# LUP-LuftbildUmweltPlanung/UNet

Measured on AMD Instinct MI355X. Metric: 512x512 tiles/sec fwd+bwd (4-ch->5-class U-Net), higher is better.
Workload: dtype f32

## Files before the change

### include/unet_hip.h

```cpp
#ifndef UNET_HIP_H
#define UNET_HIP_H

#include <stddef.h>
#include <stdint.h>

#ifdef __cplusplus
extern "C" {
#endif

#define UNET_OK 0
#define UNET_E_BADARG (-1)
#define UNET_E_UNSUPPORTED (-2)
#define UNET_E_HIP (-3)

#define UNET_ABI_VERSION 8

int unet_abi_version(void);
const char* unet_last_error(void);

#define UNET_F32 0
#define UNET_BF16 1
typedef uint16_t unet_bf16;

typedef struct {
// ... 48 lines not shown
    int ps_tail_c, ps_tail_at;
} unet_conv_desc;

int unet_conv2d_colsum_rows(const unet_conv_desc* d);
int unet_conv2d(const unet_conv_desc* d, void* stream);
size_t unet_conv2d_splitk_workspace(const unet_conv_desc* d);
int unet_conv2d_variant(const unet_conv_desc* d);
size_t unet_pack_weights_size(int Cout, int Cin, int ks, int mode);
int unet_pack_weights(const float* w, float* wp, int Cout, int Cin, int ks, int mode, void* stream);
int unet_pack_weights_strided(const float* w, long long so, long long sr, float* wp, int O, int R, void* stream);
size_t unet_pack_weights_size_bf16(int Cout, int Cin, int ks, int mode);
int unet_pack_weights_bf16(const float* w, unet_bf16* wp, int Cout, int Cin, int ks, int mode, void* stream);
typedef struct {
    const float* w;
    void* wp;
    int Cout, Cin, ks, mode;
    const float* out_scale;
} unet_pack_job;
size_t unet_pack_batch_table_bytes(int njobs);
int unet_pack_batch_build(const unet_pack_job* jobs, int njobs, int dtype, void* table_host, unsigned* total_blocks);
int unet_pack_batch_run(const void* table_dev, int njobs, unsigned total_blocks, int dtype, void* stream);
typedef struct {
    const float* x; int x_cs, x_co;
    const float* dy; int dy_cs, dy_co;
    float* dw;
    float* dbias;
    int N, IH, IW, Cin, OH, OW, Cout, ks, stride;
    float* workspace; size_t workspace_floats;
    int accumulate;
    int dtype;
    const unet_tuning* tuning;
} unet_wgrad_desc;
size_t unet_conv2d_wgrad_workspace(const unet_wgrad_desc* d);
int unet_conv2d_wgrad(const unet_wgrad_desc* d, void* stream);

int unet_bn_stats_rows(long long P);
int unet_bn_stats(const float* x, int x_cs, int x_co, long long P, int C, float* partial, void* stream);
int unet_bn_finalize(const float* psum, const float* psumsq, int rows, long long count, int C,
                     const float* gamma, const float* beta, float* running_mean, float* running_var,
                     float momentum, float eps,
                     float* scale, float* shift, float* save_mean, float* save_invstd, long long* batches_tracked, void* stream);
int unet_bn_eval_coeffs(const float* gamma, const float* beta, const float* running_mean, const float* running_var,
                        float eps, int C, float* scale, float* shift, void* stream);
int unet_affine_act(const float* x, int x_cs, int x_co, const float* scale, const float* shift,
                    const float* x2, int x2_cs, int x2_co, const float* scale2, const float* shift2,
                    float* y, int y_cs, int y_co, long long P, int C, int relu, void* stream);
int unet_bn_bwd_reduce(const float* dout, int d_cs, int d_co, const float* out, int o_cs, int o_co,
                       const float* x, int x_cs, int x_co, const float* mean, const float* invstd,
                       long long P, int C, float* partial, void* stream);
int unet_bn_bwd_finalize(const float* partial, int rows, long long count, int C,
                         float* dgamma, float* dbeta, float* c1, float* c2, void* stream);
int unet_bn_bwd_apply(const float* dout, int d_cs, int d_co, const float* out, int o_cs, int o_co,
                      const float* x, int x_cs, int x_co, const float* mean, const float* invstd,
                      const float* gamma, const float* c1, const float* c2,
                      float* dx, int dx_cs, int dx_co, float* gout, int g_cs, int g_co, int g_accumulate,
                      long long P, int C, void* stream);

int unet_maxpool3x3s2(const float* x, int x_cs, int x_co, float* y, int y_cs, int y_co, uint8_t* idx,
                      int N, int IH, int IW, int C, int OH, int OW, void* stream);
int unet_maxpool3x3s2_bwd(const float* dy, int dy_cs, int dy_co, const uint8_t* idx, float* dx, int dx_cs, int dx_co,
                          int N, int IH, int IW, int C, int OH, int OW, int accumulate, void* stream);
int unet_avgpool2_ceil(const float* x, int x_cs, int x_co, float* y, int y_cs, int y_co,
                       int N, int IH, int IW, int C, int OH, int OW, void* stream);
int unet_avgpool2_ceil_bwd(const float* dy, int dy_cs, int dy_co, float* dx, int dx_cs, int dx_co,
                           int N, int IH, int IW, int C, int OH, int OW, int accumulate, void* stream);

// ... 304 lines not shown
```

### unet_amd/_lib.py

```python
from __future__ import annotations

import ctypes as C
import os
import re
from pathlib import Path

import torch

_HERE = Path(__file__).resolve().parent
LIB_PATH = _HERE / "lib" / "libunet_hip.so"
HEADER = _HERE.parent / "include" / "unet_hip.h"

UNET_OK = 0
CONV_RELU = 1
CONV_MASK = 4
CONV_FWD = 0
CONV_DGRAD = 1
F32 = 0
BF16 = 1

c_float_p = C.POINTER(C.c_float)
vp = C.c_void_p


# ... 100 lines not shown

def _load() -> C.CDLL:
    if not LIB_PATH.exists():
        raise ImportError(
            f"{LIB_PATH} not found: build it with `python -m unet_amd.build` (hipcc --offload-arch=gfx950). "
            "The MI355X path has no CPU fallback.")
    lib = C.CDLL(str(LIB_PATH))
    missing = [s for s in declared_symbols() if not hasattr(lib, s)]
    if missing:
        raise ImportError(f"libunet_hip.so does not export: {missing}")
    return lib


lib = _load()

i, ll, f, sz = C.c_int, C.c_longlong, C.c_float, C.c_size_t
_sig = {
    "unet_abi_version": (i, []),
    "unet_last_error": (C.c_char_p, []),
    "unet_conv2d_colsum_rows": (i, [C.POINTER(ConvDesc)]),
    "unet_conv2d": (i, [C.POINTER(ConvDesc), vp]),
    "unet_conv2d_variant": (i, [C.POINTER(ConvDesc)]),
    "unet_conv2d_splitk_workspace": (sz, [C.POINTER(ConvDesc)]),
    "unet_tuning_default": (None, [C.POINTER(Tuning)]),
    "unet_pack_batch_table_bytes": (sz, [i]),
    "unet_pack_batch_build": (i, [C.POINTER(PackJob), i, i, vp, C.POINTER(C.c_uint)]),
    "unet_pack_batch_run": (i, [vp, i, C.c_uint, i, vp]),
    "unet_pack_weights_size": (sz, [i, i, i, i]),
    "unet_pack_weights": (i, [vp, vp, i, i, i, i, vp]),
    "unet_pack_weights_strided": (i, [vp, ll, ll, vp, i, i, vp]),
    "unet_row_softmax": (i, [vp, i, i, vp, i, i, ll, i, vp]),
    "unet_row_softmax_bwd": (i, [vp, i, i, vp, i, i, vp, i, i, ll, i, vp]),
    "unet_conv2d_wgrad_workspace": (sz, [C.POINTER(WgradDesc)]),
    "unet_conv2d_wgrad": (i, [C.POINTER(WgradDesc), vp]),
    "unet_bn_stats_rows": (i, [ll]),
    "unet_bn_stats": (i, [vp, i, i, ll, i, vp, vp]),
    "unet_bn_finalize": (i, [vp, vp, i, ll, i, vp, vp, vp, vp, f, f, vp, vp, vp, vp, vp, vp]),
    "unet_bn_eval_coeffs": (i, [vp, vp, vp, vp, f, i, vp, vp, vp]),
    "unet_affine_act": (i, [vp, i, i, vp, vp, vp, i, i, vp, vp, vp, i, i, ll, i, i, vp]),
    "unet_bn_bwd_reduce": (i, [vp, i, i, vp, i, i, vp, i, i, vp, vp, ll, i, vp, vp]),
    "unet_bn_bwd_finalize": (i, [vp, i, ll, i, vp, vp, vp, vp, vp]),
    "unet_bn_bwd_apply": (i, [vp, i, i, vp, i, i, vp, i, i, vp, vp, vp, vp, vp, vp, i, i, vp, i, i, i, ll, i, vp]),
    "unet_maxpool3x3s2": (i, [vp, i, i, vp, i, i, vp, i, i, i, i, i, i, vp]),
    "unet_maxpool3x3s2_bwd": (i, [vp, i, i, vp, vp, i, i, i, i, i, i, i, i, i, vp]),
    "unet_avgpool2_ceil": (i, [vp, i, i, vp, i, i, i, i, i, i, i, i, vp]),
    "unet_avgpool2_ceil_bwd": (i, [vp, i, i, vp, i, i, i, i, i, i, i, i, i, vp]),
    "unet_shuffle_blur": (i, [vp, i, i, vp, i, i, i, i, i, i, i, vp]),
    "unet_shuffle_blur_bwd": (i, [vp, i, i, vp, i, i, vp, i, i, i, i, i, i, i, vp]),
    "unet_shuffle_bwd_xmask": (i, [vp, i, i, vp, i, i, vp, i, i, i, i, i, i, vp]),
    "unet_resize_nearest": (i, [vp, i, i, vp, i, i, i, i, i, i, i, i, vp]),
    "unet_resize_nearest_bwd": (i, [vp, i, i, vp, i, i, i, i, i, i, i, i, vp]),
    "unet_nchw_to_nhwc": (i, [vp, vp, i, i, i, i, i, i, vp]),
    "unet_nhwc_to_nchw": (i, [vp, i, i, vp, i, i, i, i, vp]),
    "unet_copy_slice": (i, [vp, i, i, vp, i, i, ll, i, i, vp]),
    "unet_relu_mask": (i, [vp, i, i, vp, i, i, vp, i, i, ll, i, vp]),
    "unet_colsum": (i, [vp, i, i, ll, i, vp, vp, vp]),
    "unet_colsum_workspace": (sz, [ll, i]),
    "unet_dot": (i, [vp, i, i, vp, i, i, ll, i, vp, vp, vp]),
    "unet_ce_workspace": (sz, [ll]),
    "unet_ce_fwd": (i, [vp, i, i, vp, vp, ll, i, vp, vp, vp, vp]),
    "unet_ce_fwd_parts": (i, [vp, i, i, vp, vp, ll, i, vp, vp, vp]),
    "unet_ce_bwd": (i, [vp, i, i, vp, vp, ll, i, vp, f, vp, i, i, vp]),
    "unet_ce_fwd_pw": (i, [vp, i, i, vp, vp, ll, i, vp, vp, vp, vp]),
    "unet_ce_fwd_parts_pw": (i, [vp, i, i, vp, vp, ll, i, vp, vp, vp]),
    "unet_ce_bwd_pw": (i, [vp, i, i, vp, vp, ll, i, vp, f, vp, i, i, vp]),
    "unet_focal_fwd": (i, [vp, i, i, vp, vp, ll, i, f, vp, vp, vp]),
# ... 133 lines not shown
```

### unet_amd/csrc/conv_wgrad.hip

```cpp

#include <type_traits>
#include <utility>

#include "common.h"

namespace {

template <typename F, int... Is>
__device__ __forceinline__ void static_for_impl(F&& f, std::integer_sequence<int, Is...>) { (f(std::integral_constant<int, Is>{}), ...); }
template <int N, typename F>
__device__ __forceinline__ void static_for(F&& f) { static_for_impl(f, std::make_integer_sequence<int, N>{}); }


typedef float f32x16 __attribute__((ext_vector_type(16)));

constexpr int BK = 64;
constexpr int BC = 64;

struct WArgs {
    const float* x; const float* dy; float* part;
    float* bpart;
    int x_cs, x_co, dy_cs, dy_co;
    int N, IH, IW, Cin, Cin4, OH, OW, Cout, Cout4;
    int tiles_y, tiles_x, total_tiles, tiles_per_block;
    int kt, ct;
    int cw, nnb;
    int xcd_map;
    int csub, ksub;
};

template <int PTW, int S, int KS>
__global__ __launch_bounds__(256, 2) void wgrad_kernel(const WArgs a) {
    constexpr int PT = (S == 1) ? 64 : 32;
    constexpr int PTH = PT / PTW;
    constexpr int PAD = (KS - 1) / 2;
    constexpr int T = KS * KS;
    constexpr int HH = (PTH - 1) * S + KS, HW = (PTW - 1) * S + KS, HPIX = HH * HW;
// ... 259 lines not shown
            for (int p = 0; p < PT; ++p) bsum += dyT[p * LD + tid];
        }
#ifdef UNET_WGRAD16_NOSKIP
        compute(T1{}, T1{});
#else
        if (mv0 && nv0) {
            if (mv1 && nv1) compute(T1{}, T1{});
            else if (mv1) compute(T1{}, T0{});
            else if (nv1) compute(T0{}, T1{});
            else compute(T0{}, T0{});
        }
#endif
        __syncthreads();
    }

    if (do_bias && k0 + tid < a.Cout) a.bpart[(size_t)split * a.Cout + k0 + tid] = bsum;
    const size_t KC_ = (size_t)a.Cout * a.Cin;
    float* pb = a.part + (size_t)split * T * KC_;
#pragma unroll
    for (int i = 0; i < 2; ++i)
#pragma unroll
        for (int j = 0; j < 2; ++j) {
            const int c = c0 + wc * 32 + 16 * j + l15;
#pragma unroll
            for (int t = 0; t < T; ++t)
#pragma unroll
                for (int r = 0; r < 4; ++r) {
                    const int k = k0 + wk * 32 + 16 * i + 4 * kq + r;
                    if (k < a.Cout && c < a.Cin) pb[(size_t)t * KC_ + (size_t)k * a.Cin + c] = acc[i][j][t][r];
                }
        }
}

template <int KT, int NTW, bool SLV = false>
__global__ __launch_bounds__(256, 2) void wgrad_flat_kernel(const WArgs a) {
    constexpr int PT = 32, HW = 34, HPIX = 3 * HW, LD = 112, Q = LD / 4;
    constexpr int DIT = (PT * Q + 255) / 256, XIT = (HPIX * Q + 255) / 256;
    typedef float f32x4 __attribute__((ext_vector_type(4)));
    extern __shared__ __attribute__((aligned(16))) float smem[];
    float* dyT = smem;
    float* xh = smem + PT * LD;

    const int tid = threadIdx.x, lane = tid & 63, wave = __builtin_amdgcn_readfirstlane(tid >> 6);
    const int l15 = lane & 15, kk = lane >> 4;
    const int cols = gridDim.x;
    const int lin = blockIdx.x + cols * blockIdx.y;
    const int xcd = lin & 7, qq = lin >> 3;
    const int bx = qq % cols, split = xcd + 8 * (qq / cols);
    const int chunk = bx / a.nnb, nb = bx % a.nnb;
    const int c0 = chunk * a.cw;
    const int CW = (a.Cin - c0) < a.cw ? (a.Cin - c0) : a.cw;
    const int NTOT = 9 * CW;
    const int tile_begin = split * a.tiles_per_block;
    int tile_end = tile_begin + a.tiles_per_block;
    if (tile_end > a.total_tiles) tile_end = a.total_tiles;
    if (tile_begin >= a.total_tiles) return;

    int bfix[NTW], brow[NTW];
#pragma unroll
    for (int q = 0; q < NTW; ++q) {
        const int n = ((nb * 4 + wave) * NTW + q) * 16 + l15;
        const int nn = n < NTOT ? n : 0;
        const int t = nn / CW, c = nn - t * CW;
        const int r = t / 3, s_ = t - 3 * r;
        bfix[q] = (s_ + kk) * LD + c;
        brow[q] = r;
    }
    const int abase = kk * LD + l15;
    const int sbase = kk * LD + 16 * KT + (l15 & 3);

    f32x4 acc[KT][NTW];
    f32x4 sacc[SLV ? NTW : 1];
#pragma unroll
    for (int m = 0; m < KT; ++m)
#pragma unroll
        for (int q = 0; q < NTW; ++q) acc[m][q] = (f32x4){0.f, 0.f, 0.f, 0.f};
#pragma unroll
    for (int q = 0; q < (SLV ? NTW : 1); ++q) sacc[q] = (f32x4){0.f, 0.f, 0.f, 0.f};

    constexpr bool PF = (KT * NTW + (SLV ? NTW : 0) <= 36);
    constexpr int RIT = (HW * Q + 255) / 256;
    const int cw4 = (CW + 3) & ~3;
    struct TilePos { int oy, ox0; const float* dyb; const float* xb; };
    auto tile_pos = [&](int tile) {
        int b = tile;
        TilePos t;
        t.oy = b % a.OH; b /= a.OH;
        const int tx = b % a.tiles_x;
        const int img = b / a.tiles_x;
        t.ox0 = tx * PT;
        t.dyb = a.dy + ((size_t)img * a.OH + t.oy) * a.OW * a.dy_cs + a.dy_co;
        t.xb = a.x + (size_t)img * a.IH * a.IW * a.x_cs + a.x_co + c0;
        return t;
    };
    auto load_dy = [&](const TilePos& t, float4 (&r)[DIT]) {
#pragma unroll
        for (int it = 0; it < DIT; ++it) {
            const int e = tid + it * 256;
            const int p = e / Q, q = e - p * Q;
            const bool ok = (e < PT * Q) && (t.ox0 + p) < a.OW && 4 * q < a.Cout4;
            r[it] = ok ? *reinterpret_cast<const float4*>(t.dyb + (size_t)(t.ox0 + p) * a.dy_cs + 4 * q) : make_float4(0.f, 0.f, 0.f, 0.f);
        }
    };
    auto store_dy = [&](const float4 (&r)[DIT]) {
#pragma unroll
        for (int it = 0; it < DIT; ++it) {
            const int e = tid + it * 256;
            if (e < PT * Q) *reinterpret_cast<float4*>(dyT + e * 4) = r[it];
        }
    };
    auto load_row = [&](const TilePos& t, int hy, float4 (&r)[RIT]) {
        const int iy = t.oy - 1 + hy;
#pragma unroll
        for (int j = 0; j < RIT; ++j) {
            const int e = tid + j * 256;
            const int hx = e / Q, q = e - hx * Q;
            const int ix = t.ox0 - 1 + hx;
            const bool ok = (e < HW * Q) && iy >= 0 && iy < a.IH && ix >= 0 && ix < a.IW && 4 * q < cw4;
            r[j] = ok ? *reinterpret_cast<const float4*>(t.xb + ((size_t)iy * a.IW + ix) * a.x_cs + 4 * q) : make_float4(0.f, 0.f, 0.f, 0.f);
        }
    };
    auto store_row = [&](const TilePos& t, int hy, const float4 (&r)[RIT]) {
        float* dst = xh + ((t.oy + 2 + hy) % 3) * (HW * LD);
#pragma unroll
        for (int j = 0; j < RIT; ++j) {
            const int e = tid + j * 256;
            if (e < HW * Q) *reinterpret_cast<float4*>(dst + e * 4) = r[j];
        }
    };
    const bool do_bias = a.bpart != nullptr && bx == 0;
    float4* bred = reinterpret_cast<float4*>(smem + (PT + HPIX) * LD) + tid;
    if (do_bias) {
#pragma unroll
        for (int it = 0; it < DIT; ++it) bred[it * 256] = make_float4(0.f, 0.f, 0.f, 0.f);
    }
    auto bias_add = [&](const float4 (&r)[DIT]) {
#pragma unroll
        for (int it = 0; it < DIT; ++it) {
            float4 v = bred[it * 256];
            v.x += r[it].x; v.y += r[it].y; v.z += r[it].z; v.w += r[it].w;
            bred[it * 256] = v;
        }
    };
    auto stage_rows = [&](const TilePos& t, int hy0) {
        float4 rd[DIT];
        load_dy(t, rd);
        if (do_bias) bias_add(rd);
        store_dy(rd);
        for (int hy = hy0; hy < 3; ++hy) {
            float4 rx[RIT];
            load_row(t, hy, rx);
            store_row(t, hy, rx);
        }
    };

    int dyo[DIT], xo[RIT];
// ... 24 lines not shown
        const bool rowok = iy < a.IH;
        const float* xrow = nx.xb + (size_t)(rowok ? iy : a.IH - 1) * a.IW * a.x_cs;
#pragma unroll
        for (int it = 0; it < DIT; ++it) {
            const bool ok = dyo[it] >= 0;
            const float4 v = *reinterpret_cast<const float4*>(dyrow + (ok ? dyo[it] : ~dyo[it]));
            rdy[it] = ok ? v : make_float4(0.f, 0.f, 0.f, 0.f);
        }
#pragma unroll
        for (int j = 0; j < RIT; ++j) {
            const bool ok = xo[j] >= 0;
            const float4 v = *reinterpret_cast<const float4*>(xrow + (ok ? xo[j] : ~xo[j]));
            rxr[j] = (ok && rowok) ? v : make_float4(0.f, 0.f, 0.f, 0.f);
        }
    };

    if (tile_begin < tile_end) {
        const TilePos t0 = tile_pos(tile_begin);
        stage_rows(t0, 0);
        if (PF) strip_setup(t0);
    }
    __syncthreads();
    for (int tile = tile_begin; tile < tile_end; ++tile) {
        const int oy = tile % a.OH;
        const bool has_next = tile + 1 < tile_end;
        const bool rolling = has_next && oy + 1 < a.OH;
        TilePos nx;
        float4 pd[DIT], px[RIT];
        if (has_next) nx = tile_pos(tile + 1);
        if (PF && rolling) {
            prefetch_rolling(nx, pd, px);
            if (do_bias) bias_add(pd);
        }
        int bq[NTW];
#pragma unroll
        for (int q = 0; q < NTW; ++q) bq[q] = bfix[q] + ((oy + 2 + brow[q]) % 3) * (HW * LD);
        auto mma_step = [&](int step) {
            float av[KT], bv[NTW];
            float as_ = 0.f;
#pragma unroll
            for (int m = 0; m < KT; ++m) av[m] = dyT[abase + step * 4 * LD + m * 16];
            if constexpr (SLV) as_ = dyT[sbase + step * 4 * LD];
#pragma unroll
            for (int q = 0; q < NTW; ++q) bv[q] = xh[bq[q] + step * 4 * LD];
#pragma unroll
            for (int m = 0; m < KT; ++m)
#pragma unroll
                for (int q = 0; q < NTW; ++q) acc[m][q] = __builtin_amdgcn_mfma_f32_16x16x4f32(av[m], bv[q], acc[m][q], 0, 0, 0);
            if constexpr (SLV) {
#pragma unroll
                for (int q = 0; q < NTW; ++q) sacc[q] = __builtin_amdgcn_mfma_f32_4x4x1f32(as_, bv[q], sacc[q], 0, 0, 0);
            }
        };
        if constexpr (!PF) {
#pragma unroll 1
            for (int step = 0; step < PT / 4; ++step) mma_step(step);
        } else {
#pragma unroll 2
            for (int step = 0; step < PT / 4; ++step) mma_step(step);
        }
        if (has_next) {
            __syncthreads();
            if (PF && rolling) { store_dy(pd); store_row(nx, 2, px); }
            else {
                stage_rows(nx, rolling ? 2 : 0);
                if (PF) strip_setup(nx);
            }
            __syncthreads();
        }
    }

    if (do_bias) {
        __syncthreads();
        const float* red = smem + (PT + HPIX) * LD;
        if (tid < a.Cout) {
            float t = 0.f;
            for (int e = tid >> 2; e < PT * Q; e += Q) t += red[e * 4 + (tid & 3)];
            a.bpart[(size_t)split * a.Cout + tid] = t;
        }
    }
    const size_t KC_ = (size_t)a.Cout * a.Cin;
    float* pb = a.part + (size_t)split * 9 * KC_;
#pragma unroll
    for (int q = 0; q < NTW; ++q) {
        const int n = ((nb * 4 + wave) * NTW + q) * 16 + l15;
        if (n >= NTOT) continue;
        const int t = n / CW, c = n - t * CW;
        float* pt = pb + (size_t)t * KC_ + c0 + c;
#pragma unroll
        for (int m = 0; m < KT; ++m)
#pragma unroll
            for (int r = 0; r < 4; ++r) {
                const int k = 16 * m + 4 * kk + r;
                if (k < a.Cout) pt[(size_t)k * a.Cin] = acc[m][q][r];
            }
    }
    if constexpr (SLV) {
#pragma unroll
        for (int q = 0; q < NTW; ++q) {
            f32x4 v = sacc[q];
#pragma unroll
            for (int r = 0; r < 4; ++r) {
                v[r] += __shfl_xor(v[r], 16);
                v[r] += __shfl_xor(v[r], 32);
            }
            const int n = ((nb * 4 + wave) * NTW + q) * 16 + l15;
            if (n >= NTOT || kk != 0) continue;
            const int t = n / CW, c = n - t * CW;
            float* pt = pb + (size_t)t * KC_ + c0 + c;
#pragma unroll
            for (int r = 0; r < 4; ++r)
                if (16 * KT + r < a.Cout) pt[(size_t)(16 * KT + r) * a.Cin] = v[r];
// ... 579 lines not shown
            s2 += p[(size_t)(sp + 2 * Q) * total];
            s3 += p[(size_t)(sp + 3 * Q) * total];
        }
        for (; sp < splits; sp += Q) s0 += p[(size_t)sp * total];
    }
    ps[q][el] = (s0 + s1) + (s2 + s3);
    __syncthreads();
    if (q == 0 && e < total) {
        float s = ps[0][el];
#pragma unroll
        for (int j = 1; j < Q; ++j) s += ps[j][el];
        const size_t t = e / KC_, i = e - t * KC_;
        float* o = dw + i * T + t;
        *o = accumulate ? (*o + s) : s;
    }
}

__global__ __launch_bounds__(256) void wgrad_bias_reduce_kernel(const float* __restrict__ bpart, float* __restrict__ dbias, int splits, int Cout) {
    __shared__ double part[4][64];
    const int cl = threadIdx.x & 63, q = threadIdx.x >> 6;
    const int c = blockIdx.x * 64 + cl;
    double s = 0.0;
    if (c < Cout)
        for (int sp = q; sp < splits; sp += 4) s += (double)bpart[(size_t)sp * Cout + c];
    part[q][cl] = s;
    __syncthreads();
    if (q == 0 && c < Cout) dbias[c] = (float)(((part[0][cl] + part[1][cl]) + part[2][cl]) + part[3][cl]);
}

struct WPlan {
    unet_tuning tune;
    WArgs k;
    int ptw, splits, T, narrow, gemm1x1, small1x1, ps, bf16;
    int nsub;
    long long pix_per_block;
    size_t lds_bytes, lds_bytes16;
};

int make_wplan(const unet_wgrad_desc* d, WPlan* p) {
    UNET_CHECK_ARG(d != nullptr, "wgrad: null desc");
    p->tune = unetconv::tuning_of(d->tuning);
    UNET_CHECK_ARG(p->tune.wgrad_mfma_shape == 16 || p->tune.wgrad_mfma_shape == 32, "wgrad: unet_tuning.wgrad_mfma_shape must be 16 or 32 (start from unet_tuning_default())");
    UNET_CHECK_ARG(d->x && d->dy && d->dw, "wgrad: null tensor pointer");
    UNET_CHECK_ARG(d->ks == 1 || d->ks == 3, "wgrad: ks must be 1 or 3");
    UNET_CHECK_ARG(d->stride == 1 || d->stride == 2, "wgrad: stride must be 1 or 2");
    UNET_CHECK_ARG(!(d->ks == 1 && d->stride != 1), "wgrad: 1x1 stride 2 unsupported");
    UNET_CHECK_ARG(d->N > 0 && d->IH > 0 && d->IW > 0 && d->OH > 0 && d->OW > 0 && d->Cin > 0 && d->Cout > 0, "wgrad: bad dims");
    UNET_CHECK_ARG((long long)d->N * d->OH * d->OW < (1ll << 31), "wgrad: more than 2^31 output pixels");
    const int pad = (d->ks - 1) / 2;
    UNET_CHECK_ARG(d->OH == (d->IH + 2 * pad - d->ks) / d->stride + 1 && d->OW == (d->IW + 2 * pad - d->ks) / d->stride + 1,
                   "wgrad: output dims inconsistent");
    UNET_CHECK_ARG(d->dtype == UNET_F32 || d->dtype == UNET_BF16, "wgrad: unknown dtype %d", d->dtype);
    const int vec = d->dtype == UNET_BF16 ? 8 : 4;
    p->bf16 = d->dtype == UNET_BF16;
    UNET_CHECK_ARG(unet::slice_ok_v(d->x_cs, d->x_co, d->Cin, vec), "wgrad: bad x slice");
    UNET_CHECK_ARG(unet::slice_ok_v(d->dy_cs, d->dy_co, d->Cout, vec), "wgrad: bad dy slice");
    UNET_CHECK_ARG(unet::aligned16(d->x) && unet::aligned16(d->dy), "wgrad: x/dy must be 16-byte aligned");
    WArgs& k = p->k;
    memset(&k, 0, sizeof(k));
    k.x = d->x; k.dy = d->dy; k.part = d->workspace;
    k.x_cs = d->x_cs; k.x_co = d->x_co; k.dy_cs = d->dy_cs; k.dy_co = d->dy_co;
    k.N = d->N; k.IH = d->IH; k.IW = d->IW; k.Cin = d->Cin; k.Cin4 = unet::roundup(d->Cin, vec);
    k.OH = d->OH; k.OW = d->OW; k.Cout = d->Cout; k.Cout4 = unet::roundup(d->Cout, vec);
    p->T = d->ks * d->ks;
    p->nsub = 1;
    p->ptw = d->OW >= 32 ? 32 : (d->OW >= 16 ? 16 : 8);
    const int pt = p->bf16 ? (d->stride == 1 ? 128 : 32) : (d->stride == 1 ? 64 : 32);
    const int pth = pt / p->ptw;
    k.tiles_y = unet::cdiv(d->OH, pth);
    k.tiles_x = unet::cdiv(d->OW, p->ptw);
    k.total_tiles = d->N * k.tiles_y * k.tiles_x;
    k.kt = unet::cdiv(d->Cout, BK);
    k.ct = unet::cdiv(d->Cin, BC);
    p->narrow = (!p->bf16 && p->tune.wgrad_narrow && d->ks == 3 && d->stride == 1 && d->Cout > 80 && d->Cout <= 112 && d->OW >= 32) ? 1 : 0;
    int cols = k.kt * k.ct;
    if (p->narrow) {
        p->ptw = 32;
        k.tiles_y = d->OH;
        k.tiles_x = unet::cdiv(d->OW, 32);
        k.total_tiles = d->N * k.tiles_y * k.tiles_x;
        const int nch = unet::cdiv(d->Cin, 112);
        k.cw = unet::roundup(unet::cdiv(d->Cin, nch), 4);
        const int ntw = d->Cout > 96 ? 5 : 7;
        k.nnb = unet::cdiv(unet::cdiv(9 * k.cw, 16), 4 * ntw);
        cols = nch * k.nnb;
    }
    p->small1x1 = (!p->bf16 && d->ks == 1 && d->Cout <= 16 && k.Cin4 <= 512 && p->tune.wgrad_1x1) ? 1 : 0;
    p->ps = 1; p->pix_per_block = 0;
    if (p->small1x1) {
        const long long P = (long long)d->N * d->OH * d->OW;
        p->ps = 256 / (k.Cin4 / 4);
        {
            const int kk = 4 * ((d->Cout + 3) / 4);
            const int per_lane = (kk * k.Cin4 + kk) * (int)sizeof(float);
            if (p->ps > 65536 / per_lane) p->ps = 65536 / per_lane;
            if (p->ps < 1) p->ps = 1;
        }
        long long blocks = P / ((long long)p->ps * 64);
        if (blocks > 1024) blocks = 1024;
        if (blocks < 1) blocks = 1;
        p->pix_per_block = (P + blocks - 1) / blocks;
        p->splits = (int)((P + p->pix_per_block - 1) / p->pix_per_block);
        p->gemm1x1 = 0;
        p->lds_bytes = p->lds_bytes16 = 0;
        return UNET_OK;
    }
    p->gemm1x1 = (!p->bf16 && d->ks == 1 && p->tune.wgrad_1x1) ? 1 : 0;
    if (p->gemm1x1 && p->tune.wgrad_1x1 != 2 &&
        ((d->Cin <= 64 || d->Cout <= 64) || 2.0 * d->N * d->OH * d->OW * (double)d->Cin * d->Cout < 3.0e9))
        p->gemm1x1 = 0;
    if (p->gemm1x1) {
        k.kt = unet::cdiv(d->Cout, 128);
        k.ct = unet::cdiv(d->Cin, 128);
        k.total_tiles = unet::cdiv((long long)d->N * d->OH * d->OW, 64);
        k.tiles_y = k.tiles_x = 1;
        cols = k.kt * k.ct;
    }
    int target = 512;
// ... 83 lines not shown
    static unsigned long long configured = 0;
    if (unet::first_use_on_device(&configured)) {
        UNET_CHECK_HIP(hipFuncSetAttribute((const void*)kern, hipFuncAttributeMaxDynamicSharedMemorySize, 160 * 1024));
    }
    WArgs k = p.k;
    k.xcd_map = p.splits >= 8 ? 1 : 0;
    hipLaunchKernelGGL(kern, dim3(p.k.kt * p.k.ct, k.xcd_map ? unet::roundup(p.splits, 8) : p.splits), dim3(256), p.lds_bytes, st, k);
    UNET_CHECK_LAUNCH();
    return UNET_OK;
}

template <int PTW>
int launch_wb_ptw(const WPlan& p, int ks, int stride, hipStream_t st) {
    if (ks == 1) return launch_wb<PTW, 1, 1>(p, st);
    if (stride == 1) return launch_wb<PTW, 1, 3>(p, st);
    return launch_wb<PTW, 2, 3>(p, st);
}

template <int PTW>
int launch_w_ptw(const WPlan& p, int ks, int stride, hipStream_t st) {
    if (ks == 1) return launch_w<PTW, 1, 1>(p, st);
    if (stride == 1) return launch_w<PTW, 1, 3>(p, st);
    return launch_w<PTW, 2, 3>(p, st);
}

}

extern "C" size_t unet_conv2d_wgrad_workspace(const unet_wgrad_desc* d) {
    WPlan p;
    if (make_wplan(d, &p) != UNET_OK) return 0;
    return (size_t)p.splits * p.nsub * p.T * d->Cout * d->Cin + (size_t)p.splits * d->Cout;
}

extern "C" int unet_conv2d_wgrad(const unet_wgrad_desc* d, void* stream) {
    WPlan p;
    int rc = make_wplan(d, &p);
    if (rc != UNET_OK) return rc;
    const size_t npart = (size_t)p.splits * p.nsub * p.T * d->Cout * d->Cin;
    const size_t need = npart + (size_t)p.splits * d->Cout;
    UNET_CHECK_ARG(d->workspace != nullptr && d->workspace_floats >= need, "wgrad: workspace too small (%zu < %zu floats)",
                   d->workspace_floats, need);
    p.k.bpart = d->dbias != nullptr ? d->workspace + npart : nullptr;
    hipStream_t st = (hipStream_t)stream;
    if (p.bf16) {
        switch (p.ptw) {
            case 32: rc = launch_wb_ptw<32>(p, d->ks, d->stride, st); break;
            case 16: rc = launch_wb_ptw<16>(p, d->ks, d->stride, st); break;
            default: rc = launch_wb_ptw<8>(p, d->ks, d->stride, st); break;
        }
    } else if (p.small1x1) {
        const long long P = (long long)d->N * d->OH * d->OW;
        const dim3 grid((unsigned)p.splits);
        const int k4 = (d->Cout + 3) / 4;
        const size_t lds = (size_t)p.ps * (4 * k4 * p.k.Cin4 + 4 * k4) * sizeof(float);
        UNET_CHECK_ARG(lds <= 64 * 1024, "wgrad: head kernel needs %zu bytes of LDS", lds);
        switch (k4) {
            case 1: hipLaunchKernelGGL(wgrad1x1_small_kernel<1>, grid, dim3(256), lds, st, p.k, P, p.ps, p.pix_per_block); break;
            case 2: hipLaunchKernelGGL(wgrad1x1_small_kernel<2>, grid, dim3(256), lds, st, p.k, P, p.ps, p.pix_per_block); break;
            case 3: hipLaunchKernelGGL(wgrad1x1_small_kernel<3>, grid, dim3(256), lds, st, p.k, P, p.ps, p.pix_per_block); break;
            default: hipLaunchKernelGGL(wgrad1x1_small_kernel<4>, grid, dim3(256), lds, st, p.k, P, p.ps, p.pix_per_block); break;
        }
        UNET_CHECK_LAUNCH();
        rc = UNET_OK;
    } else if (p.gemm1x1) {
        static unsigned long long configured = 0;
        if (unet::first_use_on_device(&configured)) {
            UNET_CHECK_HIP(hipFuncSetAttribute((const void*)wgrad1x1_kernel, hipFuncAttributeMaxDynamicSharedMemorySize, 160 * 1024));
        }
        hipLaunchKernelGGL(wgrad1x1_kernel, dim3(p.k.kt * p.k.ct, p.splits), dim3(256), (size_t)2 * 64 * 128 * sizeof(float), st, p.k,
                           (long long)d->N * d->OH * d->OW);
        UNET_CHECK_LAUNCH();
        rc = UNET_OK;
    } else if (p.narrow) {
        const size_t lds = (size_t)(32 + 3 * 34) * 112 * sizeof(float) + (size_t)4 * 256 * 16;
        const dim3 grid(unet::cdiv(d->Cin, p.k.cw) * p.k.nnb, unet::roundup(p.splits, 8));
        static unsigned long long configured = 0;
        if (unet::first_use_on_device(&configured)) {
            UNET_CHECK_HIP(hipFuncSetAttribute((const void*)wgrad_flat_kernel<7, 5>, hipFuncAttributeMaxDynamicSharedMemorySize, 160 * 1024));
            UNET_CHECK_HIP(hipFuncSetAttribute((const void*)wgrad_flat_kernel<6, 5, true>, hipFuncAttributeMaxDynamicSharedMemorySize, 160 * 1024));
            UNET_CHECK_HIP(hipFuncSetAttribute((const void*)wgrad_flat_kernel<6, 7>, hipFuncAttributeMaxDynamicSharedMemorySize, 160 * 1024));
        }
        if (d->Cout > 96 && d->Cout <= 100 && p.tune.wgrad_narrow != 2) hipLaunchKernelGGL((wgrad_flat_kernel<6, 5, true>), grid, dim3(256), lds, st, p.k);
        else if (d->Cout > 96) hipLaunchKernelGGL((wgrad_flat_kernel<7, 5>), grid, dim3(256), lds, st, p.k);
        else hipLaunchKernelGGL((wgrad_flat_kernel<6, 7>), grid, dim3(256), lds, st, p.k);
        UNET_CHECK_LAUNCH();
        rc = UNET_OK;
    } else
    switch (p.ptw) {
        case 32: rc = launch_w_ptw<32>(p, d->ks, d->stride, st); break;
        case 16: rc = launch_w_ptw<16>(p, d->ks, d->stride, st); break;
        default: rc = launch_w_ptw<8>(p, d->ks, d->stride, st); break;
    }
    if (rc != UNET_OK) return rc;
    const size_t KC_ = (size_t)d->Cout * d->Cin;
    const int slices = p.splits * p.nsub;
    if (p.small1x1)
        hipLaunchKernelGGL(wgrad_reduce_rows_kernel, dim3(unet::cdiv((int)(KC_ * p.T), 64)), dim3(256), 0, st, d->workspace, d->dw,
                           p.splits, p.T, KC_, d->accumulate);
    else if (slices >= 32 && KC_ * p.T < ((size_t)1 << 31) / 8)
        hipLaunchKernelGGL(wgrad_reduce_q_kernel<8>, dim3((unsigned)unet::cdiv((long long)(KC_ * p.T), 32LL)), dim3(256), 0, st, d->workspace, d->dw,
                           slices, p.T, KC_, d->accumulate);
    else if (slices >= 8 && KC_ * p.T < ((size_t)1 << 31) / 8)
        hipLaunchKernelGGL(wgrad_reduce_q_kernel<4>, dim3((unsigned)unet::cdiv((long long)(KC_ * p.T), 64LL)), dim3(256), 0, st, d->workspace, d->dw,
                           slices, p.T, KC_, d->accumulate);
    else
        hipLaunchKernelGGL(wgrad_reduce_kernel, dim3(unet::ew_grid((long long)KC_ * p.T, 256)), dim3(256), 0, st, d->workspace, d->dw,
                           slices, p.T, KC_, d->accumulate);
    UNET_CHECK_LAUNCH();
    if (d->dbias != nullptr) {
        hipLaunchKernelGGL(wgrad_bias_reduce_kernel, dim3(unet::cdiv(d->Cout, 64)), dim3(256), 0, st, p.k.bpart, d->dbias, p.splits,
                           d->Cout);
        UNET_CHECK_LAUNCH();
    }
    return UNET_OK;
}
// ... 1 lines not shown
```

### unet_amd/ops.py

```python
from __future__ import annotations

import ctypes as C
import math
from dataclasses import dataclass
from typing import Optional

import torch

from . import _lib as L
from ._lib import ConvDesc, WgradDesc, check, lib


import contextlib
import threading

_TUNE = threading.local()


@contextlib.contextmanager
def tuning(**fields):
    prev = getattr(_TUNE, "cur", None)
    cur = L.Tuning.default() if prev is None else L.Tuning.from_buffer_copy(prev)
    for k, v in fields.items():
        if k not in dict(L.Tuning._fields_):
# ... 416 lines not shown
    d = _conv_desc(dy, wp_dgrad, dx, ks, stride, L.CONV_DGRAD, None, res, mask, False, colsum, None)
    _launch_conv(d, "conv2d_dgrad", 2.0 * dy.P * dy.C * dx.C * ks * ks)


def conv_colsum_rows(x: TS, wp, y: TS, ks, stride, kind) -> int:
    d = _conv_desc(x, wp, y, ks, stride, kind)
    r = lib.unet_conv2d_colsum_rows(C.byref(d))
    if r < 0:
        check(r, "conv2d_colsum_rows")
    return r


def _wgrad_desc(x: TS, dy: TS, dw, dbias, ks, stride, ws, accumulate) -> WgradDesc:
    d = WgradDesc()
    d.x, d.x_cs, d.x_co = x.ptr, x.cs, x.co
    d.dy, d.dy_cs, d.dy_co = dy.ptr, dy.cs, dy.co
    d.dw, d.dbias = _p(dw), _p(dbias)
    d.N, d.IH, d.IW, d.Cin = x.N, x.H, x.W, x.C
    d.OH, d.OW, d.Cout = dy.H, dy.W, dy.C
    d.ks, d.stride = ks, stride
    d.workspace = _p(ws)
    d.workspace_floats = 0 if ws is None else ws.numel()
    d.accumulate = int(accumulate)
    d.tuning = _tuning_ptr()
    assert x.bf16 == dy.bf16
    d.dtype = L.BF16 if x.bf16 else L.F32
    return d


def wgrad_workspace(x: TS, dy: TS, ks, stride, with_bias=False) -> int:
    d = _wgrad_desc(x, dy, torch.empty(0), None, ks, stride, None, 0)
    d.dw = 1
    return int(lib.unet_conv2d_wgrad_workspace(C.byref(d)))


def conv2d_wgrad(x: TS, dy: TS, dw: torch.Tensor, ks: int, stride: int, ws: torch.Tensor, dbias=None, accumulate=False):
    d = _wgrad_desc(x, dy, dw, dbias, ks, stride, ws, accumulate)
    check(lib.unet_conv2d_wgrad(C.byref(d), _stream()), "conv2d_wgrad")



def bn_stats_rows(P: int) -> int:
    return lib.unet_bn_stats_rows(P)


def bn_stats(x: TS, partial: torch.Tensor):
    check(_fn("bn_stats", x)(x.ptr, x.cs, x.co, x.P, x.C, partial.data_ptr(), _stream()), "bn_stats")


def bn_finalize(psum, psumsq, rows, count, C_, gamma, beta, rmean, rvar, momentum, eps, scale, shift, smean, sinvstd, tracked=None):
    assert tracked is None or tracked.dtype == torch.int64
    check(lib.unet_bn_finalize(_p(psum), _p(psumsq), rows, count, C_, _p(gamma), _p(beta), _p(rmean), _p(rvar), momentum, eps,
                               _p(scale), _p(shift), _p(smean), _p(sinvstd), _p(tracked), _stream()), "bn_finalize")


def bn_eval_coeffs(gamma, beta, rmean, rvar, eps, scale, shift):
    check(lib.unet_bn_eval_coeffs(_p(gamma), _p(beta), _p(rmean), _p(rvar), eps, rmean.numel(), _p(scale), _p(shift), _stream()),
          "bn_eval_coeffs")


def affine_act(x: TS, y: TS, scale=None, shift=None, x2: Optional[TS] = None, scale2=None, shift2=None, relu=False):
    check(_fn("affine_act", x)(x.ptr, x.cs, x.co, _p(scale), _p(shift),
                              None if x2 is None else x2.ptr, 0 if x2 is None else x2.cs, 0 if x2 is None else x2.co,
                              _p(scale2), _p(shift2), y.ptr, y.cs, y.co, x.P, x.C, int(relu), _stream()), "affine_act")


# ... 1443 lines not shown
```

Baseline: 148.3.

## Stream wgrad flat-kernel tiles into LDS via buffer-load-to-LDS double buffering

Adds a DMA variant of the narrow flat wgrad kernel that uses buffer_load_lds to copy dy tiles and x halo rows straight into shared memory. The dy tile is double-buffered, and only the x rows each block actually reads are fetched. The goal is to drop the register staging and explicit LDS stores of the prefetch path and overlap loads with MFMA work. In exchange it adds a plan check that decides when the row range fits, a larger LDS footprint, and raw waitcnt/barrier asm with out-of-bounds buffer addressing, which carries correctness risk.

```diff
diff --git a/include/unet_hip.h b/include/unet_hip.h
--- a/include/unet_hip.h
+++ b/include/unet_hip.h
@@ -104,6 +104,7 @@
     const unet_tuning* tuning;
 } unet_wgrad_desc;
 size_t unet_conv2d_wgrad_workspace(const unet_wgrad_desc* d);
+int unet_conv2d_wgrad_dma(const unet_wgrad_desc* d);
 int unet_conv2d_wgrad(const unet_wgrad_desc* d, void* stream);
 
 int unet_bn_stats_rows(long long P);
diff --git a/unet_amd/_lib.py b/unet_amd/_lib.py
--- a/unet_amd/_lib.py
+++ b/unet_amd/_lib.py
@@ -156,6 +156,7 @@
     "unet_row_softmax": (i, [vp, i, i, vp, i, i, ll, i, vp]),
     "unet_row_softmax_bwd": (i, [vp, i, i, vp, i, i, vp, i, i, ll, i, vp]),
     "unet_conv2d_wgrad_workspace": (sz, [C.POINTER(WgradDesc)]),
+    "unet_conv2d_wgrad_dma": (i, [C.POINTER(WgradDesc)]),
     "unet_conv2d_wgrad": (i, [C.POINTER(WgradDesc), vp]),
     "unet_bn_stats_rows": (i, [ll]),
     "unet_bn_stats": (i, [vp, i, i, ll, i, vp, vp]),
diff --git a/unet_amd/csrc/conv_wgrad.hip b/unet_amd/csrc/conv_wgrad.hip
--- a/unet_amd/csrc/conv_wgrad.hip
+++ b/unet_amd/csrc/conv_wgrad.hip
@@ -3,6 +3,7 @@
 #include <utility>
 
 #include "common.h"
+#include "wgrad_plan.h"
 
 namespace {
 
@@ -328,14 +329,15 @@
         }
 }
 
-template <int KT, int NTW, bool SLV = false>
+template <int KT, int NTW, bool SLV = false, bool DMA = false>
 __global__ __launch_bounds__(256, 2) void wgrad_flat_kernel(const WArgs a) {
     constexpr int PT = 32, HW = 34, HPIX = 3 * HW, LD = 112, Q = LD / 4;
     constexpr int DIT = (PT * Q + 255) / 256, XIT = (HPIX * Q + 255) / 256;
+    constexpr int SLOT = DMA ? 15 * 256 : HW * LD;
     typedef float f32x4 __attribute__((ext_vector_type(4)));
     extern __shared__ __attribute__((aligned(16))) float smem[];
     float* dyT = smem;
-    float* xh = smem + PT * LD;
+    float* xh = smem + (DMA ? 2 : 1) * PT * LD;
 
     const int tid = threadIdx.x, lane = tid & 63, wave = __builtin_amdgcn_readfirstlane(tid >> 6);
     const int l15 = lane & 15, kk = lane >> 4;
@@ -356,7 +358,7 @@
 #pragma unroll
     for (int q = 0; q < NTW; ++q) {
         const int n = ((nb * 4 + wave) * NTW + q) * 16 + l15;
-        const int nn = n < NTOT ? n : 0;
+        const int nn = n < NTOT ? n : (DMA ? NTOT - 1 : 0);
         const int t = nn / CW, c = nn - t * CW;
         const int r = t / 3, s_ = t - 3 * r;
         bfix[q] = (s_ + kk) * LD + c;
@@ -374,7 +376,6 @@
 #pragma unroll
     for (int q = 0; q < (SLV ? NTW : 1); ++q) sacc[q] = (f32x4){0.f, 0.f, 0.f, 0.f};
 
-    constexpr bool PF = (KT * NTW + (SLV ? NTW : 0) <= 36);
     constexpr int RIT = (HW * Q + 255) / 256;
     const int cw4 = (CW + 3) & ~3;
     struct TilePos { int oy, ox0; const float* dyb; const float* xb; };
@@ -389,6 +390,39 @@
         t.xb = a.x + (size_t)img * a.IH * a.IW * a.x_cs + a.x_co + c0;
         return t;
     };
+
+    auto mma_tile = [&](int oy, int ab, int sb) {
+        int bq[NTW];
+#pragma unroll
+        for (int q = 0; q < NTW; ++q) bq[q] = bfix[q] + ((oy + 2 + brow[q]) % 3) * SLOT;
+        auto mma_step = [&](int step) {
+            float av[KT], bv[NTW];
+            float as_ = 0.f;
+#pragma unroll
+            for (int m = 0; m < KT; ++m) av[m] = dyT[ab + step * 4 * LD + m * 16];
+            if constexpr (SLV) as_ = dyT[sb + step * 4 * LD];
+#pragma unroll
+            for (int q = 0; q < NTW; ++q) bv[q] = xh[bq[q] + step * 4 * LD];
+#pragma unroll
+            for (int m = 0; m < KT; ++m)
+#pragma unroll
+                for (int q = 0; q < NTW; ++q) acc[m][q] = __builtin_amdgcn_mfma_f32_16x16x4f32(av[m], bv[q], acc[m][q], 0, 0, 0);
+            if constexpr (SLV) {
+#pragma unroll
+                for (int q = 0; q < NTW; ++q) sacc[q] = __builtin_amdgcn_mfma_f32_4x4x1f32(as_, bv[q], sacc[q], 0, 0, 0);
+            }
+        };
+        if constexpr (KT * NTW + (SLV ? NTW : 0) > 36) {
+#pragma unroll 1
+            for (int step = 0; step < PT / 4; ++step) mma_step(step);
+        } else {
+#pragma unroll 2
+            for (int step = 0; step < PT / 4; ++step) mma_step(step);
+        }
+    };
+
+    if constexpr (!DMA) {
+    constexpr bool PF = (KT * NTW + (SLV ? NTW : 0) <= 36);
     auto load_dy = [&](const TilePos& t, float4 (&r)[DIT]) {
 #pragma unroll
         for (int it = 0; it < DIT; ++it) {
@@ -417,7 +451,7 @@
         }
     };
     auto store_row = [&](const TilePos& t, int hy, const float4 (&r)[RIT]) {
-        float* dst = xh + ((t.oy + 2 + hy) % 3) * (HW * LD);
+        float* dst = xh + ((t.oy + 2 + hy) % 3) * SLOT;
 #pragma unroll
         for (int j = 0; j < RIT; ++j) {
             const int e = tid + j * 256;
@@ -508,33 +542,7 @@
             prefetch_rolling(nx, pd, px);
             if (do_bias) bias_add(pd);
         }
-        int bq[NTW];
-#pragma unroll
-        for (int q = 0; q < NTW; ++q) bq[q] = bfix[q] + ((oy + 2 + brow[q]) % 3) * (HW * LD);
-        auto mma_step = [&](int step) {
-            float av[KT], bv[NTW];
-            float as_ = 0.f;
-#pragma unroll
-            for (int m = 0; m < KT; ++m) av[m] = dyT[abase + step * 4 * LD + m * 16];
-            if constexpr (SLV) as_ = dyT[sbase + step * 4 * LD];
-#pragma unroll
-            for (int q = 0; q < NTW; ++q) bv[q] = xh[bq[q] + step * 4 * LD];
-#pragma unroll
-            for (int m = 0; m < KT; ++m)
-#pragma unroll
-                for (int q = 0; q < NTW; ++q) acc[m][q] = __builtin_amdgcn_mfma_f32_16x16x4f32(av[m], bv[q], acc[m][q], 0, 0, 0);
-            if constexpr (SLV) {
-#pragma unroll
-                for (int q = 0; q < NTW; ++q) sacc[q] = __builtin_amdgcn_mfma_f32_4x4x1f32(as_, bv[q], sacc[q], 0, 0, 0);
-            }
-        };
-        if constexpr (!PF) {
-#pragma unroll 1
-            for (int step = 0; step < PT / 4; ++step) mma_step(step);
-        } else {
-#pragma unroll 2
-            for (int step = 0; step < PT / 4; ++step) mma_step(step);
-        }
+        mma_tile(oy, abase, sbase);
         if (has_next) {
             __syncthreads();
             if (PF && rolling) { store_dy(pd); store_row(nx, 2, px); }
@@ -545,7 +553,6 @@
             __syncthreads();
         }
     }
-
     if (do_bias) {
         __syncthreads();
         const float* red = smem + (PT + HPIX) * LD;
@@ -554,6 +561,105 @@
             for (int e = tid >> 2; e < PT * Q; e += Q) t += red[e * 4 + (tid & 3)];
             a.bpart[(size_t)split * a.Cout + tid] = t;
         }
+    }
+    } else {
+    typedef __attribute__((address_space(3))) void* lds_ptr;
+    constexpr unsigned OOB = 0x80000000u;
+    int n_lo = nb * 64 * NTW, n_hi = (n_lo + 64 * NTW < NTOT ? n_lo + 64 * NTW : NTOT) - 1;
+    if (n_lo >= NTOT) n_lo = n_hi = NTOT - 1;
+    const int rmin = n_lo / (3 * CW), rmax = n_hi / (3 * CW);
+    const int dy_row_b = (a.OW * a.dy_cs - a.dy_co) * 4, x_row_b = (a.IW * a.x_cs - a.x_co - c0) * 4;
+    unsigned dvo[DIT], xvo[RIT];
+    auto strip_setup_dma = [&](int ox0) {
+#pragma unroll
+        for (int it = 0; it < DIT; ++it) {
+            const int e = tid + it * 256;
+            const int p = e / Q, q = e - p * Q;
+            const bool ok = (e < PT * Q) && (ox0 + p) < a.OW && 4 * q < a.Cout4;
+            dvo[it] = ok ? (unsigned)((ox0 + p) * a.dy_cs + 4 * q) * 4u : OOB;
+        }
+#pragma unroll
+        for (int j = 0; j < RIT; ++j) {
+            const int e = tid + j * 256;
+            const int hx = e / Q, q = e - hx * Q;
+            const int ix = ox0 - 1 + hx;
+            const bool ok = (e < HW * Q) && ix >= 0 && ix < a.IW && 4 * q < cw4;
+            xvo[j] = ok ? (unsigned)(ix * a.x_cs + 4 * q) * 4u : OOB;
+        }
+    };
+    auto dma_dy = [&](const TilePos& t, int buf) {
+        const __amdgpu_buffer_rsrc_t rs = __builtin_amdgcn_make_buffer_rsrc(const_cast<float*>(t.dyb), 0, dy_row_b, 0x00020000);
+        float* dst = dyT + buf * (PT * LD) + wave * 256;
+#pragma unroll
+        for (int it = 0; it < DIT; ++it)
+            if (it * 256 + wave * 64 < PT * Q)
+                __builtin_amdgcn_raw_ptr_buffer_load_lds(rs, (lds_ptr)(dst + it * 1024), 16, (int)dvo[it], 0, 0, 0);
+    };
+    auto dma_row = [&](const TilePos& t, int hy) {
+        const int iy = t.oy - 1 + hy;
+        const bool rowok = iy >= 0 && iy < a.IH;
+        const __amdgpu_buffer_rsrc_t rs = __builtin_amdgcn_make_buffer_rsrc(const_cast<float*>(t.xb) + (size_t)(rowok ? iy : 0) * a.IW * a.x_cs, 0,
+                                                                            rowok ? x_row_b : 0, 0x00020000);
+        float* dst = xh + ((t.oy + 2 + hy) % 3) * SLOT + wave * 256;
+#pragma unroll
+        for (int j = 0; j < RIT; ++j)
+            if (j * 256 + wave * 64 < HW * Q)
+                __builtin_amdgcn_raw_ptr_buffer_load_lds(rs, (lds_ptr)(dst + j * 1024), 16, (int)xvo[j], 0, 0, 0);
+    };
+    auto land_and_meet = [&]() { asm volatile("s_waitcnt vmcnt(0) lgkmcnt(0)\n\ts_barrier" ::: "memory"); };
+    auto refill = [&](const TilePos& t, int buf) {
+        strip_setup_dma(t.ox0);
+        dma_dy(t, buf);
+        for (int hy = rmin; hy <= rmax; ++hy) dma_row(t, hy);
+    };
+    const bool dma_bias = a.bpart != nullptr && bx == 0;
+    float4 bsum[DIT];
+#pragma unroll
+    for (int it = 0; it < DIT; ++it) bsum[it] = make_float4(0.f, 0.f, 0.f, 0.f);
+    auto bias_add_tile = [&](int buf) {
+        const float4* src = reinterpret_cast<const float4*>(dyT + buf * (PT * LD)) + tid;
+#pragma unroll
+        for (int it = 0; it < DIT; ++it) {
+            if (it * 256 + 255 < PT * Q || tid < PT * Q - it * 256) {
+                const float4 v = src[it * 256];
+                bsum[it].x += v.x; bsum[it].y += v.y; bsum[it].z += v.z; bsum[it].w += v.w;
+            }
+        }
+    };
+    int cur = 0;
+    refill(tile_pos(tile_begin), 0);
+    land_and_meet();
+    for (int tile = tile_begin; tile < tile_end; ++tile) {
+        const int oy = tile % a.OH;
+        const bool has_next = tile + 1 < tile_end;
+        const bool rolling = has_next && oy + 1 < a.OH;
+        TilePos nx;
+        if (has_next) nx = tile_pos(tile + 1);
+        if (dma_bias) bias_add_tile(cur);
+        if (rolling) { dma_dy(nx, cur ^ 1); dma_row(nx, rmax); }
+        mma_tile(oy, abase + cur * (PT * LD), sbase + cur * (PT * LD));
+        if (has_next) {
+            if (!rolling) {
+                land_and_meet();
+                refill(nx, cur ^ 1);
+            }
+            land_and_meet();
+            cur ^= 1;
+        }
+    }
+    if (dma_bias) {
+        land_and_meet();
+        float4* red4 = reinterpret_cast<float4*>(smem) + tid;
+#pragma unroll
+        for (int it = 0; it < DIT; ++it)
+            if (it * 256 + 255 < PT * Q || tid < PT * Q - it * 256) red4[it * 256] = bsum[it];
+        land_and_meet();
+        if (tid < a.Cout) {
+            float t = 0.f;
+            for (int e = tid >> 2; e < PT * Q; e += Q) t += smem[e * 4 + (tid & 3)];
+            a.bpart[(size_t)split * a.Cout + tid] = t;
+        }
+    }
     }
     const size_t KC_ = (size_t)a.Cout * a.Cin;
     float* pb = a.part + (size_t)split * 9 * KC_;
@@ -1199,16 +1305,17 @@
     unet_tuning tune;
     WArgs k;
     int ptw, splits, T, narrow, gemm1x1, small1x1, ps, bf16;
+    int dma;
     int nsub;
     long long pix_per_block;
     size_t lds_bytes, lds_bytes16;
 };
 
-int make_wplan(const unet_wgrad_desc* d, WPlan* p) {
+int make_wplan(const unet_wgrad_desc* d, WPlan* p, bool need_dw = true) {
     UNET_CHECK_ARG(d != nullptr, "wgrad: null desc");
     p->tune = unetconv::tuning_of(d->tuning);
     UNET_CHECK_ARG(p->tune.wgrad_mfma_shape == 16 || p->tune.wgrad_mfma_shape == 32, "wgrad: unet_tuning.wgrad_mfma_shape must be 16 or 32 (start from unet_tuning_default())");
-    UNET_CHECK_ARG(d->x && d->dy && d->dw, "wgrad: null tensor pointer");
+    UNET_CHECK_ARG(d->x && d->dy && (d->dw || !need_dw), "wgrad: null tensor pointer");
     UNET_CHECK_ARG(d->ks == 1 || d->ks == 3, "wgrad: ks must be 1 or 3");
     UNET_CHECK_ARG(d->stride == 1 || d->stride == 2, "wgrad: stride must be 1 or 2");
     UNET_CHECK_ARG(!(d->ks == 1 && d->stride != 1), "wgrad: 1x1 stride 2 unsupported");
@@ -1231,6 +1338,7 @@
     k.OH = d->OH; k.OW = d->OW; k.Cout = d->Cout; k.Cout4 = unet::roundup(d->Cout, vec);
     p->T = d->ks * d->ks;
     p->nsub = 1;
+    p->dma = 0;
     p->ptw = d->OW >= 32 ? 32 : (d->OW >= 16 ? 16 : 8);
     const int pt = p->bf16 ? (d->stride == 1 ? 128 : 32) : (d->stride == 1 ? 64 : 32);
     const int pth = pt / p->ptw;
@@ -1251,6 +1359,8 @@
         const int ntw = d->Cout > 96 ? 5 : 7;
         k.nnb = unet::cdiv(unet::cdiv(9 * k.cw, 16), 4 * ntw);
         cols = nch * k.nnb;
+        p->dma = p->tune.wgrad_narrow != 4 && flat_dma_fits(d->Cin, k.cw, k.nnb, ntw) && (long long)d->IW * d->x_cs * 4 < (1ll << 31) &&
+                 (long long)d->OW * d->dy_cs * 4 < (1ll << 31);
     }
     p->small1x1 = (!p->bf16 && d->ks == 1 && d->Cout <= 16 && k.Cin4 <= 512 && p->tune.wgrad_1x1) ? 1 : 0;
     p->ps = 1; p->pix_per_block = 0;
@@ -1400,6 +1510,12 @@
     return (size_t)p.splits * p.nsub * p.T * d->Cout * d->Cin + (size_t)p.splits * d->Cout;
 }
 
+extern "C" int unet_conv2d_wgrad_dma(const unet_wgrad_desc* d) {
+    WPlan p;
+    if (make_wplan(d, &p, false) != UNET_OK) return -1;
+    return p.dma;
+}
+
 extern "C" int unet_conv2d_wgrad(const unet_wgrad_desc* d, void* stream) {
     WPlan p;
     int rc = make_wplan(d, &p);
@@ -1440,15 +1556,24 @@
         UNET_CHECK_LAUNCH();
         rc = UNET_OK;
     } else if (p.narrow) {
-        const size_t lds = (size_t)(32 + 3 * 34) * 112 * sizeof(float) + (size_t)4 * 256 * 16;
+        const size_t lds = p.dma ? (size_t)(2 * 32 * 112 + 3 * 15 * 256) * sizeof(float)
+                                 : (size_t)(32 + 3 * 34) * 112 * sizeof(float) + (size_t)4 * 256 * 16;
         const dim3 grid(unet::cdiv(d->Cin, p.k.cw) * p.k.nnb, unet::roundup(p.splits, 8));
         static unsigned long long configured = 0;
         if (unet::first_use_on_device(&configured)) {
             UNET_CHECK_HIP(hipFuncSetAttribute((const void*)wgrad_flat_kernel<7, 5>, hipFuncAttributeMaxDynamicSharedMemorySize, 160 * 1024));
             UNET_CHECK_HIP(hipFuncSetAttribute((const void*)wgrad_flat_kernel<6, 5, true>, hipFuncAttributeMaxDynamicSharedMemorySize, 160 * 1024));
             UNET_CHECK_HIP(hipFuncSetAttribute((const void*)wgrad_flat_kernel<6, 7>, hipFuncAttributeMaxDynamicSharedMemorySize, 160 * 1024));
-        }
-        if (d->Cout > 96 && d->Cout <= 100 && p.tune.wgrad_narrow != 2) hipLaunchKernelGGL((wgrad_flat_kernel<6, 5, true>), grid, dim3(256), lds, st, p.k);
+            UNET_CHECK_HIP(hipFuncSetAttribute((const void*)wgrad_flat_kernel<7, 5, false, true>, hipFuncAttributeMaxDynamicSharedMemorySize, 160 * 1024));
+            UNET_CHECK_HIP(hipFuncSetAttribute((const void*)wgrad_flat_kernel<6, 5, true, true>, hipFuncAttributeMaxDynamicSharedMemorySize, 160 * 1024));
+            UNET_CHECK_HIP(hipFuncSetAttribute((const void*)wgrad_flat_kernel<6, 7, false, true>, hipFuncAttributeMaxDynamicSharedMemorySize, 160 * 1024));
+        }
+        const bool sliver = d->Cout > 96 && d->Cout <= 100 && p.tune.wgrad_narrow != 2;
+        if (p.dma) {
+            if (sliver) hipLaunchKernelGGL((wgrad_flat_kernel<6, 5, true, true>), grid, dim3(256), lds, st, p.k);
+            else if (d->Cout > 96) hipLaunchKernelGGL((wgrad_flat_kernel<7, 5, false, true>), grid, dim3(256), lds, st, p.k);
+            else hipLaunchKernelGGL((wgrad_flat_kernel<6, 7, false, true>), grid, dim3(256), lds, st, p.k);
+        } else if (sliver) hipLaunchKernelGGL((wgrad_flat_kernel<6, 5, true>), grid, dim3(256), lds, st, p.k);
         else if (d->Cout > 96) hipLaunchKernelGGL((wgrad_flat_kernel<7, 5>), grid, dim3(256), lds, st, p.k);
         else hipLaunchKernelGGL((wgrad_flat_kernel<6, 7>), grid, dim3(256), lds, st, p.k);
         UNET_CHECK_LAUNCH();
diff --git a/unet_amd/csrc/wgrad_plan.h b/unet_amd/csrc/wgrad_plan.h
--- /dev/null
+++ b/unet_amd/csrc/wgrad_plan.h
@@ -0,0 +1,15 @@
+#pragma once
+
+inline bool flat_dma_fits(int Cin, int cw, int nnb, int ntw) {
+    const int nch = (Cin + cw - 1) / cw;
+    const int widths[2] = {nch > 1 ? cw : Cin, Cin - (nch - 1) * cw};
+    for (int CW : widths)
+        for (int nb = 0; nb < nnb; ++nb) {
+            const int lo = nb * 64 * ntw;
+            int hi = lo + 64 * ntw;
+            if (hi > 9 * CW) hi = 9 * CW;
+            if (lo >= hi) continue;
+            if ((hi - 1) / (3 * CW) - lo / (3 * CW) > 1) return false;
+        }
+    return true;
+}
diff --git a/unet_amd/ops.py b/unet_amd/ops.py
--- a/unet_amd/ops.py
+++ b/unet_amd/ops.py
@@ -472,6 +472,13 @@
     d = _wgrad_desc(x, dy, torch.empty(0), None, ks, stride, None, 0)
     d.dw = 1
     return int(lib.unet_conv2d_wgrad_workspace(C.byref(d)))
+
+
+def wgrad_uses_dma(x: TS, dy: TS, ks, stride) -> bool:
+    d = _wgrad_desc(x, dy, None, None, ks, stride, None, 0)
+    r = lib.unet_conv2d_wgrad_dma(C.byref(d))
+    assert r >= 0, "wgrad_uses_dma: bad descriptor"
+    return r == 1
 
 
 def conv2d_wgrad(x: TS, dy: TS, dw: torch.Tensor, ks: int, stride: int, ws: torch.Tensor, dbias=None, accumulate=False):
```

New measurement: 150.4 (median of 6 runs). +1.4%, better.
